# yugabyte/yugabyte-db

Hardware: NVIDIA H100
Metric: compaction GB/s (input bytes merged) (higher is better)
Workload: dtype u8

## Files before the change

yugabyte-db_b200/csrc/engine.cu:

```cuda
#include "engine.h"
#include "host_sst.h"

#include <cuda_runtime.h>
#include <algorithm>
#include <cstdio>
#include <cstring>
#include <chrono>
#include <cstdlib>
#include <mutex>

namespace ybgpu {

#define CUDA_TRY(expr)                                                                      \
  do {                                                                                      \
    cudaError_t _e = (expr);                                                                \
    if (_e != cudaSuccess) {                                                                \
      return FailCuda(#expr, _e);                                                           \
    }                                                                                       \
  } while (0)

struct RunView {
  const uint8_t* data;
  const uint64_t* blk_off;
  const uint32_t* blk_size;
// ... 396 lines not shown
  const RunView* runs;
  const uint32_t* sample_base;
  uint32_t* pos;
  unsigned long long* bucket_min;
  uint8_t* smode;
  uint32_t n_samples;
  uint32_t n_buckets;
};

constexpr unsigned long long TILE_CONT = 1ull << 63;
constexpr uint32_t SAMPLE_COARSE = 32;
__global__ void __launch_bounds__(256) k_sample_pos(PartView P, const JobParams* prm, JobDev* J, int pass) {
  const int S = prm->S, k = prm->k;
  const uint64_t total = static_cast<uint64_t>(P.n_samples) * k;
  for (uint64_t t = blockIdx.x * static_cast<uint64_t>(blockDim.x) + threadIdx.x; t < total;
       t += static_cast<uint64_t>(gridDim.x) * blockDim.x) {
    const uint32_t s = static_cast<uint32_t>(t / k), r2 = static_cast<uint32_t>(t % k);
    int r = 0;
    while (r + 1 < k && P.sample_base[r + 1] <= s) r++;
    const uint32_t s_local = s - P.sample_base[r];
    if (((s_local % SAMPLE_COARSE) == 0) != (pass == 0)) continue;
    const uint32_t idx = s_local * prm->M;
    const uint8_t* srec = P.runs[r].rec + static_cast<size_t>(idx) * S;
    const int g = group_prefix_len(srec, rec_ulen(srec, S), prm->R.enabled != 0);
    if (g < 0) { dev_fail(J, -g, s); continue; }
    bool inside = false;
    if (idx >= prm->M) {
      const uint8_t* prec = srec - static_cast<size_t>(prm->M) * S;
      inside = rec_ulen(prec, S) >= static_cast<uint32_t>(g) && common_prefix_len(srec, g, prec, g) >= static_cast<uint32_t>(g) &&
               group_prefix_len(prec, rec_ulen(prec, S), prm->R.enabled != 0) == g;
    }
    if (r2 == 0) P.smode[s] = inside ? 1 : 0;
    const RunView& q = P.runs[r2];
    uint32_t lo = 0, hi = q.n_entries;
    if (pass == 1) {
      const uint32_t c0 = s_local - s_local % SAMPLE_COARSE, c1 = c0 + SAMPLE_COARSE;
      lo = P.pos[static_cast<size_t>(P.sample_base[r] + c0) * k + r2];
      if (P.sample_base[r] + c1 < P.sample_base[r + 1]) hi = P.pos[static_cast<size_t>(P.sample_base[r] + c1) * k + r2];
    }
    if (inside) {
      if (r2 == static_cast<uint32_t>(r)) lo = hi = idx;
      while (lo < hi) {
        const uint32_t mid = (lo + hi) >> 1;
        const int c = cmp_records(q.rec + static_cast<size_t>(mid) * S, srec, S);
        if (r2 < static_cast<uint32_t>(r) ? c <= 0 : c < 0) lo = mid + 1; else hi = mid;
      }
    } else {
      while (lo < hi) {
        uint32_t mid = (lo + hi) >> 1;
        const uint8_t* c = q.rec + static_cast<size_t>(mid) * S;
        if (cmp_prefix_vs_key(srec, g, c, rec_ulen(c, S)) > 0) lo = mid + 1; else hi = mid;
      }
    }
    P.pos[static_cast<size_t>(s) * k + r2] = lo;
  }
}

__global__ void __launch_bounds__(256) k_sample_bucket(PartView P, const JobParams* prm) {
  const int k = prm->k;
  for (uint32_t s = blockIdx.x * blockDim.x + threadIdx.x; s < P.n_samples; s += gridDim.x * blockDim.x) {
    unsigned long long rank = 0;
    for (int r = 0; r < k; r++) rank += P.pos[static_cast<size_t>(s) * k + r];
    if (rank == 0) continue;
    uint32_t b = static_cast<uint32_t>(rank / prm->H);
    atomicMin(&P.bucket_min[b], (rank << 28) | s);
  }
}

__device__ __forceinline__ uint32_t block_exclusive_scan(uint32_t v, uint32_t* warp_sums, uint32_t* total) {
  const int lane = threadIdx.x & 31, wid = threadIdx.x >> 5;
  uint32_t x = v;
  for (int o = 1; o < 32; o <<= 1) { uint32_t y = __shfl_up_sync(0xffffffffu, x, o); if (lane >= o) x += y; }
  __syncthreads();
  if (lane == 31) warp_sums[wid] = x;
  __syncthreads();
  if (wid == 0) {
    uint32_t w = lane < (blockDim.x >> 5) ? warp_sums[lane] : 0;
    for (int o = 1; o < 32; o <<= 1) { uint32_t y = __shfl_up_sync(0xffffffffu, w, o); if (lane >= o) w += y; }
    warp_sums[lane] = w;
  }
  __syncthreads();
  uint32_t excl = (wid ? warp_sums[wid - 1] : 0) + x - v;
  if (total) *total = warp_sums[(blockDim.x >> 5) - 1];
  return excl;
}

constexpr int TILE_CHUNK = 2048;
__global__ void __launch_bounds__(256) k_bucket_counts(PartView P, uint32_t* partial) {
  __shared__ uint32_t sh;
  if (threadIdx.x == 0) sh = 0;
  __syncthreads();
  const uint64_t base = static_cast<uint64_t>(blockIdx.x) * TILE_CHUNK;
  uint32_t c = 0;
  for (uint32_t j = threadIdx.x; j < TILE_CHUNK; j += 256) { const uint64_t i = base + j; if (i < P.n_buckets && P.bucket_min[i] != ~0ull) c++; }
  c = __reduce_add_sync(0xffffffffu, c);
  if ((threadIdx.x & 31) == 0 && c) atomicAdd(&sh, c);
  __syncthreads();
  if (threadIdx.x == 0) partial[blockIdx.x] = sh;
}
__global__ void __launch_bounds__(256) k_build_tiles(PartView P, const JobParams* prm, const uint32_t* partial , const uint32_t* total,
                                                     uint32_t* tile_lo, unsigned long long* tile_rank, JobDev* J) {
  __shared__ uint32_t warp_sums[32];
  const int k = prm->k;
  if (blockIdx.x == 0) {
    if (threadIdx.x < k) tile_lo[threadIdx.x] = 0;
    if (threadIdx.x == 0) { tile_rank[0] = 0; J->n_tiles = *total + 1; }
  }
  const uint64_t base = static_cast<uint64_t>(blockIdx.x) * TILE_CHUNK;
  constexpr int PER = TILE_CHUNK / 256;
  unsigned long long v[PER];
  uint32_t c = 0;
  for (int j = 0; j < PER; j++) { const uint64_t i = base + threadIdx.x * PER + j; v[j] = i < P.n_buckets ? P.bucket_min[i] : ~0ull; c += v[j] != ~0ull; }
  uint32_t t = 1 + partial[blockIdx.x] + block_exclusive_scan(c, warp_sums, nullptr);
  for (int j = 0; j < PER; j++) {
    if (v[j] == ~0ull) continue;
    const uint32_t s = static_cast<uint32_t>(v[j] & ((1u << 28) - 1));
    for (int r = 0; r < k; r++) tile_lo[static_cast<size_t>(t) * k + r] = P.pos[static_cast<size_t>(s) * k + r];
    tile_rank[t] = (v[j] >> 28) | (P.smode[s] ? TILE_CONT : 0ull);
    t++;
  }
}

__global__ void __launch_bounds__(256) k_tile_check(const RunView* runs, const uint32_t* tile_lo, int k, JobDev* J) {
  const uint32_t n_tiles = J->n_tiles;
  uint32_t mx = 0;
  for (uint32_t t = blockIdx.x * blockDim.x + threadIdx.x; t < n_tiles; t += gridDim.x * blockDim.x) {
    uint32_t sz = 0;
    for (int r = 0; r < k; r++) {
      const uint32_t lo = tile_lo[static_cast<size_t>(t) * k + r];
      const uint32_t hi = (t + 1 < n_tiles) ? tile_lo[static_cast<size_t>(t + 1) * k + r] : runs[r].n_entries;
      sz += hi - lo;
    }
    mx = max(mx, sz);
  }
  mx = __reduce_max_sync(0xffffffffu, mx);
  if ((threadIdx.x & 31) == 0 && mx) atomicMax(&J->max_tile, mx);
}

struct MergeView {
  const RunView* runs;
  const uint32_t* tile_lo;
  const unsigned long long* tile_rank;
  Desc* desc;
  ValueRewrite* rewrites;
  uint32_t rewrite_cap;
  uint32_t n_tiles;
  uint16_t* fk16;
  uint32_t* fkh;
  int32_t S, k;
  uint32_t cap;
};

constexpr int MERGE_THREADS = 256;
constexpr uint8_t ENT_GROUP_START = 128;
constexpr uint32_t RW_PRE_DROPPED = 0xfffffffeu;
constexpr int RANK_C = 8;
constexpr int RANK_KMAX = 16;

namespace tile_layout {
constexpr uint32_t SEG_LO = 0;
constexpr uint32_t SEG_START = SEG_LO + 4 * MAX_RUNS;
constexpr uint32_t CBASE = SEG_START + 4 * (MAX_RUNS + 2);
constexpr uint32_t CRANK = CBASE + 4 * (MAX_RUNS + 2);
constexpr uint32_t CRANK_FIXED = 2 * (RANK_KMAX + 1) * RANK_KMAX;
constexpr uint32_t CRANK_PER = 2 * RANK_KMAX / RANK_C;
constexpr uint32_t A0 = (CRANK + CRANK_FIXED + 15) & ~15u;
constexpr uint32_t ORDER_K = CRANK_PER;
constexpr uint32_t GLEN_K = ORDER_K + 2;
constexpr uint32_t GSTART_K = GLEN_K + 2;
constexpr uint32_t A1 = A0 + 16;
constexpr uint32_t PVIS_K = GSTART_K + 2;
constexpr uint32_t RES_K = PVIS_K + 2;
constexpr uint32_t RW_K = RES_K + 1;
constexpr uint32_t PFX_K = RW_K + 4;
constexpr uint32_t PFX2_K = PFX_K + 8;
constexpr uint32_t RECS_K = PFX2_K + 8;
static_assert(RANK_KMAX % RANK_C == 0 && (PFX_K % 1) == 0, "layout");
__host__ __device__ constexpr uint32_t bytes(uint32_t S, uint32_t cap) { return A1 + (RECS_K + S + 8) * cap; }
}


static_assert(MAX_RUNS <= REPLAY_MAX_RUNS, "a replay's cursors cover every run of a job");

__device__ __noinline__ int seed_continuation(FeedState* st, const JobParams* prm, const RunView* runs, const uint32_t* seg_lo, int k, int S,
                                              const uint8_t* k0_smem) {
  ReplayRun rr[REPLAY_MAX_RUNS];
  for (int r = 0; r < k; r++) { rr[r].rec = runs[r].rec; rr[r].limit = seg_lo[r]; rr[r].data = runs[r].data; rr[r].val_off = runs[r].val_off; }
  return replay_ancestors(st, prm->R, rr, k, S, k0_smem, rec_ulen(k0_smem, S), prm->bottommost, prm->last_sequence);
}

__device__ __forceinline__ int table_id_len(const uint8_t* e, uint32_t ulen) {
  return (e[0] == 'y' || e[0] == '0') ? dockey_id_size(e, ulen) : 0;
}

__device__ __noinline__ int seed_table_from_runs(Overwrite* ow0, const JobParams* prm, const RunView* runs, const uint32_t* seg_lo,
                                                 const uint32_t* seg_start, int k, int S, const uint8_t* row, int id, bool through_tile) {
  ReplayRun rr[REPLAY_MAX_RUNS];
  for (int r = 0; r < k; r++) {
    rr[r].rec = runs[r].rec; rr[r].data = runs[r].data; rr[r].val_off = runs[r].val_off;
    rr[r].limit = seg_lo[r] + (through_tile ? seg_start[r + 1] - seg_start[r] : 0u);
  }
  FeedState st;
  const int d = replay_table_seed(&st, prm->R, rr, k, S, row, static_cast<uint32_t>(id), prm->bottommost, prm->last_sequence);
  if (d < 0) return d;
  if (!st.n_ow) return 0;
  *ow0 = st.ow[0];
  return 1;
}

__device__ __noinline__ int seed_table_in_tile(FeedState* st, const JobParams* prm, const RunView* runs, const uint8_t* recs, int SS, int S,
                                               const uint16_t* order, const uint32_t* seg_lo, const uint32_t* seg_start,
                                               uint32_t i0, uint32_t i1, const uint8_t* row, int id) {
  feed_state_reset(st);
  const uint8_t* prev = nullptr;
  for (uint32_t i = i0; i < i1; i++) {
    const uint32_t li = order[i];
    const uint8_t* c = recs + static_cast<size_t>(SS) * li;
    if (rec_flags(c, S) & REC_F_HT_FILTERED) continue;
    const uint8_t* val = nullptr;
    if (rec_vlen(c, S) && has_control_fields(rec_vfirst(c, S))) {
      int r = 0;
      while (seg_start[r + 1] <= li) r++;
      val = runs[r].data + runs[r].val_off[seg_lo[r] + (li - seg_start[r])];
    }
    const int d = replay_entry(st, prm->R, c, S, val, &prev, prm->bottommost, prm->last_sequence);
    if (d < 0) return d;
  }
  table_seed(st, row, static_cast<uint32_t>(id));
  return 0;
}

__device__ __forceinline__ uint32_t block_exclusive_max(uint32_t v, uint32_t* warp_sums) {
  const int lane = threadIdx.x & 31, wid = threadIdx.x >> 5;
  uint32_t x = v;
  for (int o = 1; o < 32; o <<= 1) { const uint32_t y = __shfl_up_sync(0xffffffffu, x, o); if (lane >= o) x = max(x, y); }
  uint32_t ex = __shfl_up_sync(0xffffffffu, x, 1);
  if (lane == 0) ex = 0;
  __syncthreads();
  if (lane == 31) warp_sums[wid] = x;
  __syncthreads();
  if (wid == 0) {
    uint32_t m = lane < (blockDim.x >> 5) ? warp_sums[lane] : 0;
    for (int o = 1; o < 32; o <<= 1) { const uint32_t y = __shfl_up_sync(0xffffffffu, m, o); if (lane >= o) m = max(m, y); }
    warp_sums[lane] = m;
  }
  __syncthreads();
  return max(wid ? warp_sums[wid - 1] : 0u, ex);
}

__global__ void __launch_bounds__(MERGE_THREADS, 3) k_merge_filter(MergeView V, const JobParams* prm, JobDev* J) {
  extern __shared__ __align__(16) uint8_t smem[];
  const int S = V.S, k = V.k;
  const int SS = S + 8;
  const uint32_t cap = V.cap;
  namespace L = tile_layout;
  uint32_t* seg_lo = reinterpret_cast<uint32_t*>(smem + L::SEG_LO);
  uint32_t* seg_start = reinterpret_cast<uint32_t*>(smem + L::SEG_START);
  uint32_t* cbase = reinterpret_cast<uint32_t*>(smem + L::CBASE);
  uint16_t* crank = reinterpret_cast<uint16_t*>(smem + L::CRANK);
  uint16_t* order = reinterpret_cast<uint16_t*>(smem + L::A0 + L::ORDER_K * cap);
  uint16_t* glen = reinterpret_cast<uint16_t*>(smem + L::A0 + L::GLEN_K * cap);
  uint16_t* gstart = reinterpret_cast<uint16_t*>(smem + L::A0 + L::GSTART_K * cap);
  uint16_t* pvis = reinterpret_cast<uint16_t*>(smem + L::A1 + L::PVIS_K * cap);
  uint8_t* res = smem + L::A1 + L::RES_K * cap;
  uint32_t* rw_slot = reinterpret_cast<uint32_t*>(smem + L::A1 + L::RW_K * cap);
  unsigned long long* pfx = reinterpret_cast<unsigned long long*>(smem + L::A1 + L::PFX_K * cap);
  unsigned long long* pfx2 = reinterpret_cast<unsigned long long*>(smem + L::A1 + L::PFX2_K * cap);
  uint8_t* recs = smem + L::A1 + L::RECS_K * cap;
  __shared__ uint32_t warp_sums[32];
  __shared__ uint32_t sh_T, sh_ngroups, sh_any_filtered, sh_any_id;
  __shared__ int sh_err;
  __shared__ uint32_t sh_c0;
  __shared__ Overwrite sh_ow0;
  __shared__ int sh_ow0_state;
  __shared__ unsigned long long sh_stats[9];
  __shared__ const uint8_t* sh_pred;
  __shared__ uint32_t sh_rb[2][MAX_RUNS + 2];

  const uint32_t tile = blockIdx.x;
  const bool cont = (V.tile_rank[tile] & TILE_CONT) != 0;
  if (threadIdx.x < 9) sh_stats[threadIdx.x] = 0;
  if (threadIdx.x < 32) {
    static_assert(MAX_RUNS <= 64, "two rounds of 32 lanes cover the runs");
    uint32_t acc = 0;
    for (int r0 = 0; r0 < k; r0 += 32) {
      const int r = r0 + static_cast<int>(threadIdx.x);
      uint32_t lo = 0, n = 0;
      if (r < k) {
        lo = V.tile_lo[static_cast<size_t>(tile) * k + r];
        const uint32_t hi = (tile + 1 < V.n_tiles) ? V.tile_lo[static_cast<size_t>(tile + 1) * k + r] : V.runs[r].n_entries;
        n = hi - lo;
      }
      uint32_t x = n;
      for (int o = 1; o < 32; o <<= 1) { const uint32_t y = __shfl_up_sync(0xffffffffu, x, o); if (static_cast<int>(threadIdx.x) >= o) x += y; }
      if (r < k) { seg_lo[r] = lo; seg_start[r] = acc + x - n; }
      acc += __shfl_sync(0xffffffffu, x, 31);
    }
    if (threadIdx.x == 0) {
      seg_start[k] = acc;
      sh_T = acc;
      sh_any_filtered = 0;
      sh_any_id = 0;
      sh_err = *reinterpret_cast<volatile int*>(&J->error);
    }
  }
  __syncthreads();
  const uint32_t T = sh_T;
  if (T == 0) return;
  if (cont && threadIdx.x == 0) atomicAdd(&J->n_cont_tiles, 1u);
  if (T > cap) { if (threadIdx.x == 0) dev_fail(J, DEV_ERR_TILE_OVERFLOW, tile); return; }

  {
    const uint32_t vpr = S >> 4;
    const uint32_t nvec = T * vpr;
    const bool vpr_pow2 = (vpr & (vpr - 1)) == 0;
    const uint32_t vpr_shift = 31 - __clz(vpr);
#pragma unroll 4
    for (uint32_t i = threadIdx.x; i < nvec; i += blockDim.x) {
      const uint32_t li = vpr_pow2 ? i >> vpr_shift : i / vpr, q = i - li * vpr;
      int r = 0;
      while (seg_start[r + 1] <= li) r++;
      const uint4 v = __ldg(reinterpret_cast<const uint4*>(V.runs[r].rec + static_cast<size_t>(seg_lo[r] + (li - seg_start[r])) * S) + q);
      uint2* d = reinterpret_cast<uint2*>(recs + static_cast<size_t>(li) * SS + 16 * q);
      d[0] = make_uint2(v.x, v.y); d[1] = make_uint2(v.z, v.w);
    }
  }
  __syncthreads();

  if (threadIdx.x < 32) {
    const uint8_t* ref = recs;
    const uint32_t ref_len = rec_ulen(ref, S);
    uint32_t c = 0xffffffffu;
    for (int r = static_cast<int>(threadIdx.x); r < k; r += 32) {
      const uint32_t n = seg_start[r + 1] - seg_start[r];
      if (!n) continue;
      const uint8_t* f = recs + static_cast<size_t>(SS) * seg_start[r];
      const uint8_t* l = recs + static_cast<size_t>(SS) * (seg_start[r + 1] - 1);
      c = min(c, min(common_prefix_len(ref, ref_len, f, rec_ulen(f, S)), common_prefix_len(ref, ref_len, l, rec_ulen(l, S))));
    }
    c = __reduce_min_sync(0xffffffffu, c);
    c = min(c, ref_len) & ~7u;
    if (c + 16 > static_cast<uint32_t>(S - 16)) c = (S - 16 >= 16) ? static_cast<uint32_t>(S - 32) & ~7u : 0;
    if (threadIdx.x == 0) sh_c0 = c;
  }
  if (threadIdx.x == 0) {
    const uint8_t* pred = nullptr;
    if (cont) {
      for (int r = 0; r < k; r++) {
        uint32_t j = seg_lo[r];
        const uint8_t* c2 = nullptr;
        while (j > 0) {
          const uint8_t* q = V.runs[r].rec + static_cast<size_t>(j - 1) * S;
          if (!(rec_flags(q, S) & REC_F_INVISIBLE)) { c2 = q; break; }
          j--;
        }
        if (c2 && (!pred || cmp_records(c2, pred, S) >= 0)) pred = c2;
      }
    }
    sh_pred = pred;
  }
  __syncthreads();
  {
    const uint32_t c0 = sh_c0;
    for (uint32_t li = threadIdx.x; li < T; li += blockDim.x)
    {
      pfx[li] = bswap64(ld_u64_aligned(recs + static_cast<size_t>(SS) * li + c0));
      pfx2[li] = bswap64(ld_u64_aligned(recs + static_cast<size_t>(SS) * li + c0 + 8));
    }
  }
  __syncthreads();

  {
    constexpr int MT = 2;
    uint16_t* bufs[2] = {order, reinterpret_cast<uint16_t*>(crank)};
    auto le = [&](uint32_t a, uint32_t b) -> bool {
      const unsigned long long pa = pfx[a], pb = pfx[b];
      if (pa != pb) return pa < pb;
      const unsigned long long qa = pfx2[a], qb = pfx2[b];
      if (qa != qb) return qa < qb;
      return cmp_records(recs + static_cast<size_t>(SS) * a, recs + static_cast<size_t>(SS) * b, S) <= 0;
    };
    for (uint32_t li = threadIdx.x; li < T; li += blockDim.x) bufs[0][li] = static_cast<uint16_t>(li);
    if (threadIdx.x <= static_cast<uint32_t>(k)) sh_rb[0][threadIdx.x] = seg_start[threadIdx.x];
    __syncthreads();
    int nruns = k, cur = 0;
    while (nruns > 1) {
      const uint16_t* src = bufs[cur]; uint16_t* dst = bufs[cur ^ 1];
      const uint32_t* rb = sh_rb[cur];
      const int npairs = (nruns + 1) >> 1;
      for (uint32_t o0 = threadIdx.x * MT; o0 < T; o0 += blockDim.x * MT) {
        int p = 0;
        while (p + 1 < npairs && rb[2 * (p + 1)] <= o0) p++;
        uint32_t a0 = rb[2 * p], a1 = rb[min(2 * p + 1, nruns)], b1 = rb[min(2 * p + 2, nruns)];
        const uint32_t d = o0 - a0, la = a1 - a0, lb = b1 - a1;
        uint32_t lo = d > lb ? d - lb : 0, hi = min(d, la);
        while (lo < hi) {
          const uint32_t mid = (lo + hi) >> 1;
          if (le(src[a0 + mid], src[a1 + (d - 1 - mid)])) lo = mid + 1; else hi = mid;
        }
        uint32_t i = a0 + lo, j = a1 + (d - lo);
        const uint32_t o_end = min(o0 + MT, T);
        for (uint32_t o = o0; o < o_end; o++) {
          while (o == b1 && p + 1 < npairs) {
            p++;
            a0 = rb[2 * p]; a1 = rb[min(2 * p + 1, nruns)]; b1 = rb[min(2 * p + 2, nruns)];
            i = a0; j = a1;
          }
          uint16_t pick;
          if (i < a1 && (j >= b1 || le(src[i], src[j]))) pick = src[i++]; else pick = src[j++];
          dst[o] = pick;
        }
      }
      if (threadIdx.x <= static_cast<uint32_t>(npairs)) sh_rb[cur ^ 1][threadIdx.x] = rb[min(2 * static_cast<int>(threadIdx.x), nruns)];
      __syncthreads();
      nruns = npairs; cur ^= 1;
    }
    if (cur) {
      for (uint32_t li = threadIdx.x; li < T; li += blockDim.x) order[li] = bufs[1][li];
    }
  }
  for (uint32_t li = threadIdx.x; li < T; li += blockDim.x) {
    int r = 0;
    while (seg_start[r + 1] <= li) r++;
    const uint32_t p = li - seg_start[r];
    const uint8_t* e = recs + static_cast<size_t>(SS) * li;
    if (p > 0 && cmp_records(e - SS, e, S) >= 0) { dev_fail(J, DEV_ERR_UNSORTED, tile); sh_err = 1; }
    int fk = 0;
    const int g = group_prefix_len(e, rec_ulen(e, S), prm->R.enabled != 0, V.fk16 ? &fk : nullptr);
    if (g < 0) { dev_fail(J, -g, tile); sh_err = 1; glen[li] = 0; } else glen[li] = static_cast<uint16_t>(g);
    if (V.fk16) {
      const uint32_t gid = V.runs[r].gid_base + seg_lo[r] + p;
      V.fk16[gid] = static_cast<uint16_t>(g < 0 ? 0 : fk);
      if (V.fkh) V.fkh[gid] = (g < 0 || fk <= 0) ? 0u : leveldb_hash(e, static_cast<uint32_t>(fk), kBloomSeed);
    }
    if (rec_flags(e, S) & REC_F_INVISIBLE) sh_any_filtered = 1;
    if (e[0] == 'y' || e[0] == '0') sh_any_id = 1;
  }
  __syncthreads();
  if (sh_err) return;

  if (sh_any_filtered) {
    if (threadIdx.x == 0) {
      uint32_t last = 0xffff;
      for (uint32_t i = 0; i < T; i++) {
        pvis[i] = static_cast<uint16_t>(last);
        if (!(rec_flags(recs + static_cast<size_t>(SS) * (order[i]), S) & REC_F_INVISIBLE)) last = i;
      }
    }
  } else {
    for (uint32_t i = threadIdx.x; i < T; i += blockDim.x) pvis[i] = static_cast<uint16_t>(i ? i - 1 : 0xffff);
  }
  __syncthreads();

  const uint32_t items = (T + blockDim.x - 1) / blockDim.x;
  uint32_t my_groups = 0;
  unsigned long long st_counted = 0, st_hidden = 0, st_obsolete = 0, st_in_k = 0, st_in_v = 0;
  for (uint32_t j = 0; j < items; j++) {
    const uint32_t i = threadIdx.x * items + j;
    if (i >= T) break;
    const uint32_t li = order[i];
    const uint8_t* e = recs + static_cast<size_t>(SS) * (li);
    uint8_t f = 0;
    if (!(rec_flags(e, S) & REC_F_INVISIBLE)) {
      f |= ENT_COUNTED; st_counted++;
      st_in_k += rec_ulen(e, S) + 8; st_in_v += rec_vlen(e, S);
      const uint64_t suffix = rec_suffix(e, S);
      const uint32_t type = static_cast<uint32_t>(suffix & 0xff);
      const uint64_t seq = suffix >> 8;
      if (type != 0 && type != 1) dev_fail(J, DEV_ERR_UNSUPPORTED_VALUE, tile);
      const uint32_t ulen = rec_ulen(e, S);
      bool first_occ = true;
      if (pvis[i] != 0xffff) {
        const uint8_t* pe = recs + static_cast<size_t>(SS) * (order[pvis[i]]);
        first_occ = cmp_user_keys(pe, rec_ulen(pe, S), e, ulen) != 0;
      } else if (cont && sh_pred) {
        first_occ = cmp_user_keys(sh_pred, rec_ulen(sh_pred, S), e, ulen) != 0;
      }
      if (!first_occ) { f |= ENT_DROP_HIDDEN; st_hidden++; }
      else if (type == 0 && prm->bottommost && seq <= prm->last_sequence) { f |= ENT_DROP_OBSOLETE; st_obsolete++; }
      else {
        f |= ENT_KEEP;
        if (prm->bottommost && seq < prm->last_sequence) {
          bool is_largest = ulen == prm->largest_len;
          for (uint32_t q = 0; is_largest && q < ulen; q++) is_largest = e[q] == prm->largest[q];
          if (!is_largest) f |= ENT_ZERO_SEQ;
        }
      }
    }
    bool gs = i == 0;
    if (!gs) {
      const uint32_t lp = order[i - 1];
      const uint32_t g = glen[li];
      gs = glen[lp] != g || common_prefix_len(e, g, recs + static_cast<size_t>(SS) * (lp), g) < g;
    }
    if (gs) { my_groups++; f |= ENT_GROUP_START; }
    res[i] = f;
  }
  uint32_t ngroups;
  uint32_t gbase = block_exclusive_scan(my_groups, warp_sums, &ngroups);
  for (uint32_t j = 0; j < items; j++) {
    const uint32_t i = threadIdx.x * items + j;
    if (i >= T) break;
    if (res[i] & ENT_GROUP_START) gstart[gbase++] = static_cast<uint16_t>(i);
  }
  if (threadIdx.x == 0) { gstart[ngroups] = static_cast<uint16_t>(T); sh_ngroups = ngroups; }
  __syncthreads();

  unsigned long long st_feed = 0;
  for (uint32_t i = threadIdx.x; i < T; i += blockDim.x) {
    uint32_t mark = 0xffffffffu;
    if (i > 0 && prm->R.enabled && (res[i] & ENT_KEEP) && (res[i - 1] & ENT_KEEP)) {
      const uint8_t* e = recs + static_cast<size_t>(SS) * order[i];
      const uint8_t* p = recs + static_cast<size_t>(SS) * order[i - 1];
      const uint32_t ul = rec_ulen(e, S), pl = rec_ulen(p, S);
      const uint32_t hl = doc_ht_len_from_end(e, ul), hp = doc_ht_len_from_end(p, pl);
      if (hl && hp && ul - hl == pl - hp &&
          !(rec_vlen(e, S) && rec_vfirst(e, S) == 'k') && !(rec_vlen(p, S) && rec_vfirst(p, S) == 'k')) {
        const EncHt& chosen = (e[0] == 'y' && prm->R.has_cotables_cutoff) ? prm->R.cotables_cutoff_enc : prm->R.cutoff_enc;
        if (encht_cmp(p + pl - hp, hp, chosen.b, chosen.n) <= 0 && common_prefix_len(e, ul - hl, p, ul - hl) >= ul - hl)
          mark = RW_PRE_DROPPED;
      }
    }
    rw_slot[i] = mark;
  }
  const bool ids = prm->R.enabled && sh_any_id;
  if (ids) {
    const uint32_t ngroups = sh_ngroups;
    if (threadIdx.x == 0) {
      int state = 0;
      const uint8_t* e = recs + static_cast<size_t>(SS) * order[0];
      const uint32_t ul = rec_ulen(e, S);
      const int id = table_id_len(e, ul);
      if (id > 0 && static_cast<uint32_t>(id) < ul) {
        bool lookup = e[id] != '!';
        if (!lookup && cont && ngroups > 1) {
          const uint8_t* n1 = recs + static_cast<size_t>(SS) * order[gstart[1]];
          lookup = rec_ulen(n1, S) > static_cast<uint32_t>(id) && n1[id] != '!' && common_prefix_len(n1, id, e, id) >= static_cast<uint32_t>(id);
        }
        if (lookup) {
          const int rc = seed_table_from_runs(&sh_ow0, prm, V.runs, seg_lo, seg_start, k, S, e, id, e[id] == '!');
          if (rc < 0) dev_fail(J, -rc, tile);
          state = rc > 0 ? 2 : 1;
        }
      }
      sh_ow0_state = state;
    }
    const uint32_t per = (ngroups + blockDim.x - 1) / blockDim.x;
    const uint32_t g0 = min(threadIdx.x * per, ngroups), g1 = min(g0 + per, ngroups);
    uint32_t last = 0;
    for (uint32_t g = g0; g < g1; g++) {
      bool head = g == 0;
      if (!head) {
        const uint8_t* e = recs + static_cast<size_t>(SS) * order[gstart[g]];
        const uint8_t* p = recs + static_cast<size_t>(SS) * order[gstart[g - 1]];
        const int id = table_id_len(e, rec_ulen(e, S));
        head = id <= 0 || table_id_len(p, rec_ulen(p, S)) != id || common_prefix_len(p, id, e, id) < static_cast<uint32_t>(id);
      }
      if (head) last = g + 1;
      pvis[g] = static_cast<uint16_t>(last ? last - 1 : 0xffff);
    }
    const uint32_t carry = block_exclusive_max(last, warp_sums);
    for (uint32_t g = g0; g < g1 && pvis[g] == 0xffff; g++) pvis[g] = static_cast<uint16_t>(carry - 1);
  }
  __syncthreads();
  if (prm->R.enabled) {
    for (uint32_t g = threadIdx.x; g < sh_ngroups; g += blockDim.x) {
      FeedState st;
      feed_state_reset(&st);
      const uint32_t i0 = gstart[g], i1 = gstart[g + 1];
      if (ids) {
        const uint8_t* e0 = recs + static_cast<size_t>(SS) * order[i0];
        const uint32_t ul0 = rec_ulen(e0, S);
        const int id = table_id_len(e0, ul0);
        if (id > 0 && static_cast<uint32_t>(id) < ul0 && e0[id] != '!') {
          const uint32_t h = pvis[g];
          if (h == 0 && sh_ow0_state) {
            if (sh_ow0_state == 2) feed_state_seed(&st, e0, id, sh_ow0);
          } else if (recs[static_cast<size_t>(SS) * order[gstart[h]] + id] == '!') {
            const int rc = seed_table_in_tile(&st, prm, V.runs, recs, SS, S, order, seg_lo, seg_start, gstart[h], gstart[h + 1], e0, id);
            if (rc < 0) { dev_fail(J, -rc, tile); continue; }
          }
        }
      }
      const bool continued = cont && g == 0;
      if (continued) {
        const int rc = seed_continuation(&st, prm, V.runs, seg_lo, k, S, recs + static_cast<size_t>(SS) * order[i0]);
        if (rc < 0) { dev_fail(J, -rc, tile); continue; }
      }
      {
        bool all_above = !(prm->R.lower_len | prm->R.upper_len) && !continued;
        for (uint32_t i = i0; i < i1 && all_above; i++) {
          if (!(res[i] & ENT_KEEP)) continue;
          const uint8_t* e = recs + static_cast<size_t>(SS) * (order[i]);
          const uint32_t ulen = rec_ulen(e, S);
          const uint8_t b0 = ulen ? e[0] : 10;
          const uint32_t htl = doc_ht_len_from_end(e, ulen);
          const uint8_t vf = rec_vfirst(e, S);
          if (b0 == 10 || b0 == 6 || b0 == 7 || b0 == 'y' || b0 == '0' || !htl ||
              encht_cmp(e + ulen - htl, htl, prm->R.cutoff_enc.b, prm->R.cutoff_enc.n) <= 0 ||
              (rec_vlen(e, S) && (has_control_fields(vf) || vf == 'z' || vf == '|')))
            all_above = false;
        }
        if (all_above) continue;
      }
      for (uint32_t i = i0; i < i1; i++) {
        uint8_t f = res[i];
        if (!(f & ENT_KEEP)) continue;
        if (rw_slot[i] == RW_PRE_DROPPED) { rw_slot[i] = 0xffffffffu; res[i] = f & ~ENT_KEEP & ~ENT_ZERO_SEQ; st_feed++; continue; }
        const uint32_t li = order[i];
        const uint8_t* e = recs + static_cast<size_t>(SS) * (li);
        int r = 0;
        while (seg_start[r + 1] <= li) r++;
        const uint32_t idx = seg_lo[r] + (li - seg_start[r]);
        const uint32_t vlen = rec_vlen(e, S);
        const uint8_t vfirst = rec_vfirst(e, S);
        const uint8_t* val = nullptr;
        if (vlen && has_control_fields(vfirst)) val = V.runs[r].data + V.runs[r].val_off[idx];
        ValueRewrite rw;
        int d = feed_step(&st, prm->R, e, rec_ulen(e, S), vfirst, val, vlen, &rw);
        if (d < 0) { dev_fail(J, -d, tile); break; }
        if (d == 0) { res[i] = f & ~ENT_KEEP & ~ENT_ZERO_SEQ; st_feed++; continue; }
        f |= static_cast<uint8_t>(d);
        if (d & ENT_VAL_REENCODE) {
          uint32_t slot = atomicAdd(&J->n_rewrites, 1u);
          if (slot < V.rewrite_cap) { V.rewrites[slot] = rw; rw_slot[i] = slot; }
          else dev_fail(J, DEV_ERR_UNSUPPORTED_VALUE, tile);
        }
        res[i] = f;
      }
    }
  }
  if (prm->R.enabled) {
    for (uint32_t g = threadIdx.x; g < sh_ngroups; g += blockDim.x) {
      const uint32_t i0 = gstart[g], i1 = gstart[g + 1];
      bool done = false;
      for (uint32_t i = i0; i < i1; i++) {
        uint8_t f = res[i] & static_cast<uint8_t>(~ENT_FIRST_OF_ROW);
        if (!done && (f & ENT_KEEP)) { f |= ENT_FIRST_OF_ROW; done = true; }
        res[i] = f;
      }
    }
  }
  __syncthreads();

  const unsigned long long rank0 = V.tile_rank[tile] & ~TILE_CONT;
  unsigned long long st_kept = 0, st_kbytes = 0, st_vbytes = 0, mn = ~0ull, mx = 0;
  for (uint32_t i = threadIdx.x; i < T; i += blockDim.x) {
    const uint32_t li = order[i];
    const uint8_t* e = recs + static_cast<size_t>(SS) * (li);
    int r = 0;
    while (seg_start[r + 1] <= li) r++;
    const uint32_t idx = seg_lo[r] + (li - seg_start[r]);
    const uint8_t f = res[i];
    Desc d;
    d.gid = V.runs[r].gid_base + idx;
    d.klen = static_cast<uint16_t>(rec_ulen(e, S) + 8);
    d.flags = prm->R.enabled ? f : (f & static_cast<uint8_t>(~ENT_GROUP_START)); d.run = static_cast<uint8_t>(r);
    d.rewrite_slot = rw_slot[i];
    uint32_t vout = rec_vlen(e, S);
    if (f & ENT_VAL_TOMBSTONE) vout = 1;
    else if (f & ENT_VAL_REENCODE) { const ValueRewrite& rw = V.rewrites[rw_slot[i]]; vout = vout - rw.skip + rw.prefix_len; }
    d.vlen_out = vout;
    if ((f & ENT_KEEP) && !(f & ENT_VAL_REENCODE)) {
      uint32_t sh = 0xffffu;
      int j = static_cast<int>(i) - 1;
      for (int steps = 0; j >= 0 && !(res[j] & ENT_KEEP) && steps < 24; steps++) j--;
      if (j >= 0 && (res[j] & ENT_KEEP)) {
        const uint8_t* p = recs + static_cast<size_t>(SS) * order[j];
        const uint32_t m = min(rec_ulen(e, S), rec_ulen(p, S));
        const uint32_t c = common_prefix_len(e, m, p, m);
        if (c < m) sh = c;
      }
      d.rewrite_slot = sh;
    }
    V.desc[rank0 + i] = d;
    if (f & ENT_KEEP) {
      st_kept++; st_kbytes += d.klen; st_vbytes += vout;
      if ((rec_suffix(e, S) & 0xff) != 1) atomicAdd(&J->n_kept_deletions, 1ull);
      const unsigned long long seq = (f & ENT_ZERO_SEQ) ? 0ull : (rec_suffix(e, S) >> 8);
      mn = min(mn, seq); mx = max(mx, seq);
    }
  }
  unsigned long long vals[9] = {st_counted, st_hidden, st_obsolete, st_feed, st_kept, st_kbytes, st_vbytes, st_in_k, st_in_v};
  for (int q = 0; q < 9; q++) {
    unsigned long long v = vals[q];
    if (__any_sync(0xffffffffu, (v >> 26) != 0)) {
      for (int o = 16; o; o >>= 1) v += __shfl_xor_sync(0xffffffffu, v, o);
    } else {
      v = __reduce_add_sync(0xffffffffu, static_cast<unsigned>(v));
    }
    if ((threadIdx.x & 31) == 0 && v) atomicAdd(&sh_stats[q], v);
  }
  for (int o = 16; o; o >>= 1) { mn = min(mn, __shfl_xor_sync(0xffffffffu, mn, o)); mx = max(mx, __shfl_xor_sync(0xffffffffu, mx, o)); }
  if ((threadIdx.x & 31) == 0) { if (mn != ~0ull) atomicMin(&J->min_seq, mn); if (mx) atomicMax(&J->max_seq, mx); }
  __syncthreads();
  if (threadIdx.x == 0) {
    if (sh_stats[0]) atomicAdd(&J->n_counted, sh_stats[0]);
    if (sh_stats[1]) atomicAdd(&J->n_hidden, sh_stats[1]);
    if (sh_stats[2]) atomicAdd(&J->n_obsolete, sh_stats[2]);
    if (sh_stats[3]) atomicAdd(&J->n_feed_dropped, sh_stats[3]);
    if (sh_stats[4]) atomicAdd(&J->n_kept, sh_stats[4]);
    if (sh_stats[5]) atomicAdd(&J->out_key_bytes, sh_stats[5]);
    if (sh_stats[6]) atomicAdd(&J->out_val_bytes, sh_stats[6]);
    if (sh_stats[7]) atomicAdd(&J->in_key_bytes, sh_stats[7]);
    if (sh_stats[8]) atomicAdd(&J->in_val_bytes, sh_stats[8]);
  }
}

constexpr int EMIT_CHUNK = 2048;
constexpr int EMIT_THREADS = 256;

struct Sums3 { unsigned long long n, kb, vb; };

__global__ void __launch_bounds__(EMIT_THREADS) k_emit_sums(const Desc* desc, uint64_t N, Sums3* partial) {
  __shared__ unsigned long long sh[3];
  if (threadIdx.x < 3) sh[threadIdx.x] = 0;
  __syncthreads();
  const uint64_t base = static_cast<uint64_t>(blockIdx.x) * EMIT_CHUNK;
  unsigned long long n = 0, kb = 0, vb = 0;
  for (uint32_t j = threadIdx.x; j < EMIT_CHUNK; j += blockDim.x) {
    uint64_t i = base + j;
    if (i < N) { Desc d = desc[i]; if (d.flags & ENT_KEEP) { n++; kb += d.klen; vb += d.vlen_out; } }
  }
  for (int o = 16; o; o >>= 1) { n += __shfl_xor_sync(0xffffffffu, n, o); kb += __shfl_xor_sync(0xffffffffu, kb, o); vb += __shfl_xor_sync(0xffffffffu, vb, o); }
  if ((threadIdx.x & 31) == 0) { atomicAdd(&sh[0], n); atomicAdd(&sh[1], kb); atomicAdd(&sh[2], vb); }
  __syncthreads();
  if (threadIdx.x == 0) { partial[blockIdx.x].n = sh[0]; partial[blockIdx.x].kb = sh[1]; partial[blockIdx.x].vb = sh[2]; }
}

__global__ void __launch_bounds__(1024) k_scan_sums(Sums3* partial, uint32_t n) {
  __shared__ unsigned long long ws[3][32];
  __shared__ unsigned long long carry[3];
  if (threadIdx.x < 3) carry[threadIdx.x] = 0;
  __syncthreads();
  const int lane = threadIdx.x & 31, wid = threadIdx.x >> 5;
  for (uint32_t base = 0; base < n; base += 1024) {
    uint32_t i = base + threadIdx.x;
    unsigned long long v[3] = {0, 0, 0};
    if (i < n) { v[0] = partial[i].n; v[1] = partial[i].kb; v[2] = partial[i].vb; }
    unsigned long long x[3] = {v[0], v[1], v[2]};
    for (int q = 0; q < 3; q++) {
      for (int o = 1; o < 32; o <<= 1) { unsigned long long y = __shfl_up_sync(0xffffffffu, x[q], o); if (lane >= o) x[q] += y; }
      if (lane == 31) ws[q][wid] = x[q];
    }
    __syncthreads();
    if (wid == 0) {
      for (int q = 0; q < 3; q++) {
        unsigned long long w = ws[q][lane];
        for (int o = 1; o < 32; o <<= 1) { unsigned long long y = __shfl_up_sync(0xffffffffu, w, o); if (lane >= o) w += y; }
        ws[q][lane] = w;
      }
    }
    __syncthreads();
    if (i < n) {
      partial[i].n = carry[0] + (wid ? ws[0][wid - 1] : 0) + x[0] - v[0];
      partial[i].kb = carry[1] + (wid ? ws[1][wid - 1] : 0) + x[1] - v[1];
      partial[i].vb = carry[2] + (wid ? ws[2][wid - 1] : 0) + x[2] - v[2];
    }
    __syncthreads();
    if (threadIdx.x < 3) carry[threadIdx.x] += ws[threadIdx.x][31];
    __syncthreads();
  }
}

__device__ __forceinline__ void warp_copy(uint8_t* dst, const uint8_t* src, uint32_t n, int lane) {
  uint32_t head = (4 - (reinterpret_cast<uintptr_t>(dst) & 3)) & 3;
  if (head > n) head = n;
  if (lane < static_cast<int>(head)) dst[lane] = src[lane];
  dst += head; src += head; n -= head;
  const uint32_t nw = n >> 2;
  const uint32_t sh = reinterpret_cast<uintptr_t>(src) & 3;
  const uint32_t* s32 = reinterpret_cast<const uint32_t*>(src - sh);
  uint32_t* d32 = reinterpret_cast<uint32_t*>(dst);
  for (uint32_t w = lane; w < nw; w += 32) {
    uint32_t lo = __ldg(s32 + w);
    if (sh) { uint32_t hi = __ldg(s32 + w + 1); lo = __funnelshift_r(lo, hi, sh * 8); }
    d32[w] = lo;
  }
  const uint32_t tail = n & 3;
  if (lane < static_cast<int>(tail)) dst[nw * 4 + lane] = src[nw * 4 + lane];
}

struct EmitView {
  const RunView* runs;
  const Desc* desc;
  const Sums3* partial;
  const ValueRewrite* rewrites;
  uint8_t* out_keys; uint64_t* out_koff;
  uint8_t* out_vals; uint64_t* out_voff;
  uint64_t N;
};

__global__ void __launch_bounds__(EMIT_THREADS) k_emit(EmitView E, int S, JobDev* J) {
  __shared__ uint32_t s_n[EMIT_CHUNK + 1];
  __shared__ uint32_t s_kb[EMIT_CHUNK + 1];
  __shared__ uint32_t s_vb[EMIT_CHUNK + 1];
  __shared__ uint32_t warp_sums[32];
  const uint64_t base = static_cast<uint64_t>(blockIdx.x) * EMIT_CHUNK;
  const Sums3 off = E.partial[blockIdx.x];
  constexpr int PER = EMIT_CHUNK / EMIT_THREADS;
  uint32_t n = 0, kb = 0, vb = 0;
  uint32_t ln[PER], lk[PER], lv[PER];
  for (int j = 0; j < PER; j++) {
    uint64_t i = base + threadIdx.x * PER + j;
    ln[j] = n; lk[j] = kb; lv[j] = vb;
    if (i < E.N) { Desc d = E.desc[i]; if (d.flags & ENT_KEEP) { n++; kb += d.klen; vb += d.vlen_out; } }
  }
  uint32_t bn = block_exclusive_scan(n, warp_sums, nullptr);
  uint32_t bk = block_exclusive_scan(kb, warp_sums, nullptr);
  uint32_t bv = block_exclusive_scan(vb, warp_sums, nullptr);
  for (int j = 0; j < PER; j++) {
    uint32_t q = threadIdx.x * PER + j;
    s_n[q] = bn + ln[j]; s_kb[q] = bk + lk[j]; s_vb[q] = bv + lv[j];
  }
  __syncthreads();
  const int lane = threadIdx.x & 31, wid = threadIdx.x >> 5;
  for (uint32_t q = wid; q < EMIT_CHUNK; q += EMIT_THREADS / 32) {
    const uint64_t i = base + q;
    if (i >= E.N) break;
    const Desc d = E.desc[i];
    if (!(d.flags & ENT_KEEP)) continue;
    const RunView& run = E.runs[d.run];
    const uint32_t idx = d.gid - run.gid_base;
    const uint8_t* rec = run.rec + static_cast<size_t>(idx) * S;
    const uint64_t j = off.n + s_n[q];
    const uint64_t ko = off.kb + s_kb[q], vo = off.vb + s_vb[q];
    if (lane == 0) { E.out_koff[j] = ko; E.out_voff[j] = vo; }
    const uint32_t ulen = d.klen - 8u;
    uint8_t* kd = E.out_keys + ko;
    for (uint32_t b = lane; b < ulen; b += 32) kd[b] = rec[b];
    if (lane < 8) {
      uint64_t suffix = rec_suffix(rec, S);
      if (d.flags & ENT_ZERO_SEQ) suffix &= 0xff;
      kd[ulen + lane] = static_cast<uint8_t>(suffix >> (8 * lane));
    }
    uint8_t* vd = E.out_vals + vo;
    const uint8_t* vs = run.data + run.val_off[idx];
    if (d.flags & ENT_VAL_TOMBSTONE) {
      if (lane == 0) vd[0] = 'X';
    } else if (d.flags & ENT_VAL_REENCODE) {
      const ValueRewrite& rw = E.rewrites[d.rewrite_slot];
      if (lane < rw.prefix_len) vd[lane] = rw.prefix[lane];
      const uint32_t rest = d.vlen_out - rw.prefix_len;
      for (uint32_t b = lane; b < rest; b += 32) vd[rw.prefix_len + b] = vs[rw.skip + b];
    } else {
      warp_copy(vd, vs, d.vlen_out, lane);
    }
  }
  (void)J;
}

__device__ __forceinline__ unsigned long long mix64(unsigned long long x) {
  x ^= x >> 33; x *= 0xff51afd7ed558ccdull; x ^= x >> 33; x *= 0xc4ceb9fe1a85ec53ull; x ^= x >> 33; return x;
}
__global__ void __launch_bounds__(256) k_digest(const uint8_t* keys, const uint64_t* koff, const uint8_t* vals,
                                                const uint64_t* voff, uint64_t n, JobDev* J) {
  unsigned long long acc = 0;
  for (uint64_t i = blockIdx.x * static_cast<uint64_t>(blockDim.x) + threadIdx.x; i < n;
// ... 1611 lines not shown
```

Baseline: 274.3.

## Stage merge records with cp.async, skip all-above groups early, batch stats atomics

The global-to-shared record staging loop now issues 8-byte cp.async copies instead of 16-byte register loads followed by split stores. The run-index search also carries over between iterations. The group-level 'all entries above cutoff' check moves before feed-state setup and continuation seeding, so those groups skip that work. Per-thread atomics for kept deletions and min/max sequence, plus the shared-memory stat atomics, are replaced by per-warp shared slots that a few threads reduce and then publish with one atomic each. Smaller 8-byte async copies mean more copy instructions per record, and the earlier skip adds a check for groups that are not skipped.

New measurement: 283.8 (median of 6 runs). 1.03x the previous value.

```diff
diff --git a/profiles/merge_measure.py b/profiles/merge_measure.py
--- /dev/null
+++ b/profiles/merge_measure.py
@@ -0,0 +1,96 @@
+import argparse
+import importlib
+import json
+import os
+import statistics
+import subprocess
+import sys
+import tempfile
+
+import torch
+
+ROOT = os.path.dirname(os.path.dirname(os.path.abspath(__file__)))
+sys.path[:0] = [ROOT]
+pkg = importlib.import_module("yugabyte-db_b200")
+
+ap = argparse.ArgumentParser()
+ap.add_argument("--rows", type=int, default=40000000, help="entries per shape")
+ap.add_argument("--steps", type=int, default=5)
+ap.add_argument("--warmup", type=int, default=2)
+ap.add_argument("--shapes", default="bench,mvcc")
+ap.add_argument("--trace-dir", default=None, help="where the chrome traces are written (default: a temporary directory)")
+args = ap.parse_args()
+if args.steps < 1 or args.warmup < 1:
+    raise SystemExit("--steps and --warmup must be at least 1")
+if not torch.cuda.is_available() or pkg.device_count() < 1:
+    raise SystemExit("merge_measure.py needs a CUDA device: kernel times cannot be taken without one")
+print(subprocess.run(["nvidia-smi", "--query-gpu=name,power.limit,clocks.max.sm", "--format=csv,noheader"],
+                     capture_output=True, text=True).stdout.strip())
+trace_dir = args.trace_dir or tempfile.mkdtemp(prefix="merge_measure_")
+os.makedirs(trace_dir, exist_ok=True)
+stream = torch.cuda.current_stream().cuda_stream
+
+
+def shape_inputs(name):
+    versions = 20 if name == "mvcc" else 1
+    cfg = pkg.GenConfig(seed=2, num_rows=args.rows // versions, cols=1, versions=versions, num_files=8, value_len=256)
+    kw = {"filter_policy": 1}
+    if name == "mvcc":
+        kw["cutoff_ht"] = (cfg.base_micros + 18 * 1000 + 500) << 12
+    return pkg.generate_ssts(cfg, max_threads=8), kw
+
+
+def measure(name):
+    ssts, kw = shape_inputs(name)
+    handles = [pkg.sst_block_handles(s.meta_view())[:2] for s in ssts]
+    dev_files = []
+    for s in ssts:
+        v = s.data_view()
+        t = torch.zeros(v.size + 64, dtype=torch.uint8, device="cuda")
+        t[16:16 + v.size].copy_(torch.from_numpy(v))
+        dev_files.append(t)
+    torch.cuda.synchronize()
+
+    def one_job():
+        job = pkg.GpuCompactionJob(verify_checksums=True, cuda_stream=stream, **kw)
+        for t, s, (off, sz) in zip(dev_files, ssts, handles):
+            job.add_input_device(t.data_ptr() + 16, s.data_view().size, off, sz)
+        st = job.run()
+        torch.cuda.synchronize()
+        job.close()
+        return st
+
+    for _ in range(args.warmup):
+        one_job()
+    stats = [one_job() for _ in range(args.steps)]
+    with torch.profiler.profile(activities=[torch.profiler.ProfilerActivity.CUDA]) as prof:
+        for _ in range(args.steps):
+            one_job()
+    path = os.path.join(trace_dir, "merge_measure_%s_trace.json" % name)
+    prof.export_chrome_trace(path)
+    with open(path) as f:
+        kern = [e for e in json.load(f)["traceEvents"] if e.get("ph") == "X" and e.get("cat") == "kernel" and "k_merge_filter" in e["name"]]
+    if len(kern) != args.steps:
+        raise SystemExit("%s: expected %d k_merge_filter launches in the trace, found %d" % (name, args.steps, len(kern)))
+
+    st = stats[-1]
+    n = st.num_input_records
+    ikey = st.total_input_raw_key_bytes / n
+    S = max(32, (int(round(ikey)) - 8 + 16 + 15) & ~15)
+    moved = n * (S + 16 + 2 + 4)
+    merge_ms = [s.phase_seconds[3] * 1e3 for s in stats]
+    kern_ms = [e["dur"] / 1e3 for e in kern]
+    tiles = kern[-1].get("args", {}).get("grid", ["not recorded"])[0]
+    print("\n%s: %d entries in, %d out; record stride %d B; %s tiles (k_merge_filter grid)" % (name, n, st.num_output_records, S, tiles))
+    print("  merge phase, CUDA events, per job:    %s ms (median %.3f)" % (" ".join("%.3f" % x for x in merge_ms), statistics.median(merge_ms)))
+    print("  k_merge_filter, torch.profiler:       %s ms (median %.3f)" % (" ".join("%.3f" % x for x in kern_ms), statistics.median(kern_ms)))
+    print("  bytes it must move: %.3f GB; at the median kernel time %.0f GB/s" % (moved / 1e9, moved / statistics.median(kern_ms) / 1e6))
+    print("  job device time (gpu_seconds), per job: %s ms" % " ".join("%.2f" % (s.gpu_seconds * 1e3) for s in stats))
+    del dev_files
+    torch.cuda.empty_cache()
+
+
+for shape in args.shapes.split(","):
+    if shape not in ("bench", "mvcc"):
+        raise SystemExit("unknown shape %r" % shape)
+    measure(shape)
diff --git a/yugabyte-db_b200/csrc/engine.cu b/yugabyte-db_b200/csrc/engine.cu
--- a/yugabyte-db_b200/csrc/engine.cu
+++ b/yugabyte-db_b200/csrc/engine.cu
@@ -572,6 +572,7 @@
 };
 
 constexpr int MERGE_THREADS = 256;
+constexpr int MERGE_STATS = 12;
 constexpr uint8_t ENT_GROUP_START = 128;
 constexpr uint32_t RW_PRE_DROPPED = 0xfffffffeu;
 constexpr int RANK_C = 8;
@@ -648,6 +649,32 @@
   }
   table_seed(st, row, static_cast<uint32_t>(id));
   return 0;
+}
+
+__device__ __forceinline__ unsigned long long warp_sum_u64(unsigned long long v) {
+  if (__any_sync(0xffffffffu, (v >> 26) != 0)) {
+    for (int o = 16; o; o >>= 1) v += __shfl_xor_sync(0xffffffffu, v, o);
+    return v;
+  }
+  return __reduce_add_sync(0xffffffffu, static_cast<unsigned>(v));
+}
+
+__device__ __forceinline__ bool group_all_above(const JobParams* prm, const uint8_t* recs, int SS, int S, const uint16_t* order,
+                                                const uint8_t* res, uint32_t i0, uint32_t i1) {
+  if (prm->R.lower_len | prm->R.upper_len) return false;
+  for (uint32_t i = i0; i < i1; i++) {
+    if (!(res[i] & ENT_KEEP)) continue;
+    const uint8_t* e = recs + static_cast<size_t>(SS) * (order[i]);
+    const uint32_t ulen = rec_ulen(e, S);
+    const uint8_t b0 = ulen ? e[0] : 10;
+    const uint32_t htl = doc_ht_len_from_end(e, ulen);
+    const uint8_t vf = rec_vfirst(e, S);
+    if (b0 == 10 || b0 == 6 || b0 == 7 || b0 == 'y' || b0 == '0' || !htl ||
+        encht_cmp(e + ulen - htl, htl, prm->R.cutoff_enc.b, prm->R.cutoff_enc.n) <= 0 ||
+        (rec_vlen(e, S) && (has_control_fields(vf) || vf == 'z' || vf == '|')))
+      return false;
+  }
+  return true;
 }
 
 __device__ __forceinline__ uint32_t block_exclusive_max(uint32_t v, uint32_t* warp_sums) {
@@ -693,13 +720,12 @@
   __shared__ uint32_t sh_c0;
   __shared__ Overwrite sh_ow0;
   __shared__ int sh_ow0_state;
-  __shared__ unsigned long long sh_stats[9];
+  __shared__ unsigned long long sh_stats[MERGE_THREADS / 32][MERGE_STATS];
   __shared__ const uint8_t* sh_pred;
   __shared__ uint32_t sh_rb[2][MAX_RUNS + 2];
 
   const uint32_t tile = blockIdx.x;
   const bool cont = (V.tile_rank[tile] & TILE_CONT) != 0;
-  if (threadIdx.x < 9) sh_stats[threadIdx.x] = 0;
   if (threadIdx.x < 32) {
     static_assert(MAX_RUNS <= 64, "two rounds of 32 lanes cover the runs");
     uint32_t acc = 0;
@@ -731,19 +757,19 @@
   if (T > cap) { if (threadIdx.x == 0) dev_fail(J, DEV_ERR_TILE_OVERFLOW, tile); return; }
 
   {
-    const uint32_t vpr = S >> 4;
-    const uint32_t nvec = T * vpr;
-    const bool vpr_pow2 = (vpr & (vpr - 1)) == 0;
-    const uint32_t vpr_shift = 31 - __clz(vpr);
-#pragma unroll 4
-    for (uint32_t i = threadIdx.x; i < nvec; i += blockDim.x) {
-      const uint32_t li = vpr_pow2 ? i >> vpr_shift : i / vpr, q = i - li * vpr;
-      int r = 0;
+    const uint32_t wpr = S >> 3;
+    const uint32_t nw = T * wpr;
+    const bool wpr_pow2 = (wpr & (wpr - 1)) == 0;
+    const uint32_t wpr_shift = 31 - __clz(wpr);
+    const uint32_t recs_s = static_cast<uint32_t>(__cvta_generic_to_shared(recs));
+    int r = 0;
+    for (uint32_t i = threadIdx.x; i < nw; i += blockDim.x) {
+      const uint32_t li = wpr_pow2 ? i >> wpr_shift : i / wpr, q = i - li * wpr;
       while (seg_start[r + 1] <= li) r++;
-      const uint4 v = __ldg(reinterpret_cast<const uint4*>(V.runs[r].rec + static_cast<size_t>(seg_lo[r] + (li - seg_start[r])) * S) + q);
-      uint2* d = reinterpret_cast<uint2*>(recs + static_cast<size_t>(li) * SS + 16 * q);
-      d[0] = make_uint2(v.x, v.y); d[1] = make_uint2(v.z, v.w);
-    }
+      const uint8_t* src = V.runs[r].rec + static_cast<size_t>(seg_lo[r] + (li - seg_start[r])) * S + 8 * q;
+      asm volatile("cp.async.ca.shared.global [%0], [%1], 8;" ::"r"(recs_s + li * SS + 8 * q), "l"(src) : "memory");
+    }
+    asm volatile("cp.async.wait_all;" ::: "memory");
   }
   __syncthreads();
 
@@ -924,6 +950,12 @@
     if (res[i] & ENT_GROUP_START) gstart[gbase++] = static_cast<uint16_t>(i);
   }
   if (threadIdx.x == 0) { gstart[ngroups] = static_cast<uint16_t>(T); sh_ngroups = ngroups; }
+  const int lane = threadIdx.x & 31, wid = threadIdx.x >> 5;
+  {
+    const unsigned long long c0 = warp_sum_u64(st_counted), c1 = warp_sum_u64(st_hidden), c2 = warp_sum_u64(st_obsolete),
+                             c7 = warp_sum_u64(st_in_k), c8 = warp_sum_u64(st_in_v);
+    if (lane == 0) { sh_stats[wid][0] = c0; sh_stats[wid][1] = c1; sh_stats[wid][2] = c2; sh_stats[wid][7] = c7; sh_stats[wid][8] = c8; }
+  }
   __syncthreads();
 
   unsigned long long st_feed = 0;
@@ -985,9 +1017,11 @@
   __syncthreads();
   if (prm->R.enabled) {
     for (uint32_t g = threadIdx.x; g < sh_ngroups; g += blockDim.x) {
+      const uint32_t i0 = gstart[g], i1 = gstart[g + 1];
+      const bool continued = cont && g == 0;
+      if (!ids && !continued && group_all_above(prm, recs, SS, S, order, res, i0, i1)) continue;
       FeedState st;
       feed_state_reset(&st);
-      const uint32_t i0 = gstart[g], i1 = gstart[g + 1];
       if (ids) {
         const uint8_t* e0 = recs + static_cast<size_t>(SS) * order[i0];
         const uint32_t ul0 = rec_ulen(e0, S);
@@ -1002,26 +1036,11 @@
           }
         }
       }
-      const bool continued = cont && g == 0;
       if (continued) {
         const int rc = seed_continuation(&st, prm, V.runs, seg_lo, k, S, recs + static_cast<size_t>(SS) * order[i0]);
         if (rc < 0) { dev_fail(J, -rc, tile); continue; }
-      }
-      {
-        bool all_above = !(prm->R.lower_len | prm->R.upper_len) && !continued;
-        for (uint32_t i = i0; i < i1 && all_above; i++) {
-          if (!(res[i] & ENT_KEEP)) continue;
-          const uint8_t* e = recs + static_cast<size_t>(SS) * (order[i]);
-          const uint32_t ulen = rec_ulen(e, S);
-          const uint8_t b0 = ulen ? e[0] : 10;
-          const uint32_t htl = doc_ht_len_from_end(e, ulen);
-          const uint8_t vf = rec_vfirst(e, S);
-          if (b0 == 10 || b0 == 6 || b0 == 7 || b0 == 'y' || b0 == '0' || !htl ||
-              encht_cmp(e + ulen - htl, htl, prm->R.cutoff_enc.b, prm->R.cutoff_enc.n) <= 0 ||
-              (rec_vlen(e, S) && (has_control_fields(vf) || vf == 'z' || vf == '|')))
-            all_above = false;
-        }
-        if (all_above) continue;
+      } else if (ids && group_all_above(prm, recs, SS, S, order, res, i0, i1)) {
+        continue;
       }
       for (uint32_t i = i0; i < i1; i++) {
         uint8_t f = res[i];
@@ -1064,7 +1083,7 @@
   __syncthreads();
 
   const unsigned long long rank0 = V.tile_rank[tile] & ~TILE_CONT;
-  unsigned long long st_kept = 0, st_kbytes = 0, st_vbytes = 0, mn = ~0ull, mx = 0;
+  unsigned long long st_kept = 0, st_kbytes = 0, st_vbytes = 0, st_kdel = 0, mn = ~0ull, mx = 0;
   for (uint32_t i = threadIdx.x; i < T; i += blockDim.x) {
     const uint32_t li = order[i];
     const uint8_t* e = recs + static_cast<size_t>(SS) * (li);
@@ -1096,34 +1115,36 @@
     V.desc[rank0 + i] = d;
     if (f & ENT_KEEP) {
       st_kept++; st_kbytes += d.klen; st_vbytes += vout;
-      if ((rec_suffix(e, S) & 0xff) != 1) atomicAdd(&J->n_kept_deletions, 1ull);
+      st_kdel += (rec_suffix(e, S) & 0xff) != 1;
       const unsigned long long seq = (f & ENT_ZERO_SEQ) ? 0ull : (rec_suffix(e, S) >> 8);
       mn = min(mn, seq); mx = max(mx, seq);
     }
   }
-  unsigned long long vals[9] = {st_counted, st_hidden, st_obsolete, st_feed, st_kept, st_kbytes, st_vbytes, st_in_k, st_in_v};
-  for (int q = 0; q < 9; q++) {
-    unsigned long long v = vals[q];
-    if (__any_sync(0xffffffffu, (v >> 26) != 0)) {
-      for (int o = 16; o; o >>= 1) v += __shfl_xor_sync(0xffffffffu, v, o);
-    } else {
-      v = __reduce_add_sync(0xffffffffu, static_cast<unsigned>(v));
-    }
-    if ((threadIdx.x & 31) == 0 && v) atomicAdd(&sh_stats[q], v);
+  {
+    const unsigned long long c3 = warp_sum_u64(st_feed), c4 = warp_sum_u64(st_kept), c5 = warp_sum_u64(st_kbytes),
+                             c6 = warp_sum_u64(st_vbytes), c9 = warp_sum_u64(st_kdel);
+    if (lane == 0) { sh_stats[wid][3] = c3; sh_stats[wid][4] = c4; sh_stats[wid][5] = c5; sh_stats[wid][6] = c6; sh_stats[wid][9] = c9; }
   }
   for (int o = 16; o; o >>= 1) { mn = min(mn, __shfl_xor_sync(0xffffffffu, mn, o)); mx = max(mx, __shfl_xor_sync(0xffffffffu, mx, o)); }
-  if ((threadIdx.x & 31) == 0) { if (mn != ~0ull) atomicMin(&J->min_seq, mn); if (mx) atomicMax(&J->max_seq, mx); }
+  if (lane == 0) { sh_stats[wid][MERGE_STATS - 2] = mn; sh_stats[wid][MERGE_STATS - 1] = mx; }
   __syncthreads();
-  if (threadIdx.x == 0) {
-    if (sh_stats[0]) atomicAdd(&J->n_counted, sh_stats[0]);
-    if (sh_stats[1]) atomicAdd(&J->n_hidden, sh_stats[1]);
-    if (sh_stats[2]) atomicAdd(&J->n_obsolete, sh_stats[2]);
-    if (sh_stats[3]) atomicAdd(&J->n_feed_dropped, sh_stats[3]);
-    if (sh_stats[4]) atomicAdd(&J->n_kept, sh_stats[4]);
-    if (sh_stats[5]) atomicAdd(&J->out_key_bytes, sh_stats[5]);
-    if (sh_stats[6]) atomicAdd(&J->out_val_bytes, sh_stats[6]);
-    if (sh_stats[7]) atomicAdd(&J->in_key_bytes, sh_stats[7]);
-    if (sh_stats[8]) atomicAdd(&J->in_val_bytes, sh_stats[8]);
+  if (threadIdx.x < MERGE_STATS) {
+    const int q = threadIdx.x;
+    unsigned long long v = sh_stats[0][q];
+    for (int w = 1; w < MERGE_THREADS / 32; w++) {
+      const unsigned long long x = sh_stats[w][q];
+      v = q == MERGE_STATS - 2 ? min(v, x) : q == MERGE_STATS - 1 ? max(v, x) : v + x;
+    }
+    unsigned long long* dst;
+    switch (q) {
+      case 0: dst = &J->n_counted; break;       case 1: dst = &J->n_hidden; break;      case 2: dst = &J->n_obsolete; break;
+      case 3: dst = &J->n_feed_dropped; break;  case 4: dst = &J->n_kept; break;        case 5: dst = &J->out_key_bytes; break;
+      case 6: dst = &J->out_val_bytes; break;   case 7: dst = &J->in_key_bytes; break;  case 8: dst = &J->in_val_bytes; break;
+      case 9: dst = &J->n_kept_deletions; break; case 10: dst = &J->min_seq; break;    default: dst = &J->max_seq; break;
+    }
+    if (q == MERGE_STATS - 2) { if (v != ~0ull) atomicMin(dst, v); }
+    else if (q == MERGE_STATS - 1) { if (v) atomicMax(dst, v); }
+    else if (v) atomicAdd(dst, v);
   }
 }
 
```
